# jlvdb/yet_another_wizz

Measured on AMD Instinct MI355X. Metric: candidate pairs/s, higher is better.
Workload: dtype f64

## Files before the change

### yet_another_wizz_amd/csrc/yawhip.hip

```cpp

#include <hip/hip_runtime.h>

#include <algorithm>
#include <numeric>
#include <chrono>
#include <climits>
#include <cmath>
#include <cstdio>
#include <cstdlib>
#include <cstring>
#include <memory>
#include <new>
#include <string>
#include <type_traits>
#include <utility>
#include <functional>
#include <vector>

#include "yawhip_internal.h"

using namespace yawhip_detail;

namespace {
constexpr int WG = 256;
constexpr int STAGE = 256;
constexpr int MSTAGE = 64;
constexpr int MAX_EDGES = 512;
constexpr int BAND_MIN_STREAM_RUN = 64;
constexpr int64_t SYNC_GRID_MIN_ITEMS = 400000;
constexpr int MAX_STRIP_REACH = 12;
constexpr int COUNT_FLUSH_MASK = (1 << 13) - 1;
constexpr int MERGED_FLUSH_MASK = (1 << 16) - 1;
constexpr double PAD_COORD = 4.0;

struct alignas(16) Obj {
    double x, y, z, w;
};

struct alignas(16) ObjF {
    float x, y, z, pad;
};

constexpr double FILTER_GUARD = 8.0 * 5.9604644775390625e-8;

inline double sep_angle(double rwin) { return 2.0 * std::asin(std::min(1.0, 0.5 * (rwin + 2e-9))); }

__device__ __forceinline__ double cap_lo64(double u, double c, double s) {
    const double ul = fmax(u - 1e-9, -1.0);
    return ul <= -c + 1e-12 ? -1.0 - 2e-9 : fma(ul, c, -sqrt(fmax(fma(-ul, ul, 1.0), 0.0)) * s) - 2e-9;
}
__device__ __forceinline__ double cap_hi64(double u, double c, double s) {
    const double uh = fmin(u + 1e-9, 1.0);
// ... 739 lines not shown
           (band_small_hist(weighted, nslots, hp) ? 0 : (size_t)nslots * hp * (weighted ? 8 : 4)) + 16;
}
typedef __attribute__((address_space(3))) unsigned char lds_byte;
__device__ __forceinline__ __attribute__((address_space(3))) void *lds_ptr(unsigned addr) { return (__attribute__((address_space(3))) void *)(size_t)addr; }
__device__ __forceinline__ double lds_f64(unsigned addr) { return *(const __attribute__((address_space(3))) double *)(size_t)addr; }
__device__ __forceinline__ int lds_i32(unsigned addr) { return *(const __attribute__((address_space(3))) int *)(size_t)addr; }

__device__ __forceinline__ int wave_max_nonneg(int v) {
    v = max(v, __builtin_amdgcn_update_dpp(0, v, 0x111, 0xf, 0xf, false));
    v = max(v, __builtin_amdgcn_update_dpp(0, v, 0x112, 0xf, 0xf, false));
    v = max(v, __builtin_amdgcn_update_dpp(0, v, 0x114, 0xf, 0xf, false));
    v = max(v, __builtin_amdgcn_update_dpp(0, v, 0x118, 0xf, 0xf, false));
    v = max(v, __builtin_amdgcn_update_dpp(0, v, 0x142, 0xa, 0xf, false));
    v = max(v, __builtin_amdgcn_update_dpp(0, v, 0x143, 0xc, 0xf, false));
    return __builtin_amdgcn_readlane(v, 63);
}

__device__ __forceinline__ unsigned int wave_sum_lane63(unsigned int v) {
    v += (unsigned int)__builtin_amdgcn_update_dpp(0, (int)v, 0x111, 0xf, 0xf, false);
    v += (unsigned int)__builtin_amdgcn_update_dpp(0, (int)v, 0x112, 0xf, 0xf, false);
    v += (unsigned int)__builtin_amdgcn_update_dpp(0, (int)v, 0x114, 0xf, 0xf, false);
    v += (unsigned int)__builtin_amdgcn_update_dpp(0, (int)v, 0x118, 0xf, 0xf, false);
    v += (unsigned int)__builtin_amdgcn_update_dpp(0, (int)v, 0x142, 0xa, 0xf, false);
    v += (unsigned int)__builtin_amdgcn_update_dpp(0, (int)v, 0x143, 0xc, 0xf, false);
    return v;
}

template <int R, int CAP, bool WEIGHTED, int NE, bool MERGED, bool UNI>
__global__ __launch_bounds__(64) void k_count_band(const DevTab *__restrict__ tabs, const Item *__restrict__ items, int n_bins,
                                                   int n_edges, const double *__restrict__ t,
                                                   const double *__restrict__ rwin_k, unsigned flush_mask, int hp_shift,
                                                   int batch_log2, unsigned long long *__restrict__ out_counts,
                                                   double *__restrict__ partials,
                                                   unsigned long long *__restrict__ counters) {
    using HistT = typename std::conditional<WEIGHTED, double, unsigned int>::type;
    constexpr bool NF1 = NE == 2;
    constexpr bool REG_EDGES = NE >= 2 && (!MERGED || UNI);
    constexpr bool NEED_THR = !REG_EDGES;
    constexpr int HB = WEIGHTED ? 3 : 2;
    using L = BandLds<CAP>;
    constexpr int LDS_X = L::X, LDS_K = L::K, LDS_Y = L::Y, LDS_H = L::H, LDS_Z = L::Z, LDS_H_BYTES = L::H_BYTES, BCOL = L::COL;
    __shared__ __attribute__((aligned(16))) unsigned char lds_fix[L::FIXED];
    extern __shared__ __attribute__((aligned(16))) unsigned char lds_dyn[];
    const int nkb = MERGED ? n_bins : 1;
    const int nf = NF1 ? 1 : n_edges - 1;
    const int nslots = nkb * nf;
    const int hp = 1 << hp_shift;
    double *sx = reinterpret_cast<double *>(lds_fix + LDS_X);
    double *sy = reinterpret_cast<double *>(lds_fix + LDS_Y);
    double *sz = reinterpret_cast<double *>(lds_fix + LDS_Z);
    int *sk = reinterpret_cast<int *>(lds_fix + LDS_K);
    unsigned char *p = lds_dyn;
    double *sw = reinterpret_cast<double *>(p); if (WEIGHTED) p += BCOL;
    constexpr bool ROW1 = !(MERGED && !UNI);
    const int thr_rows = ROW1 ? 1 : nkb;
    double *thr = reinterpret_cast<double *>(p); if (NEED_THR) p += (size_t)thr_rows * n_edges * sizeof(double);
    const bool small_hist = band_small_hist(WEIGHTED, nslots, hp);
    HistT *hist = reinterpret_cast<HistT *>(small_hist ? lds_fix + LDS_H : p);
    unsigned int *dummy = reinterpret_cast<unsigned int *>(lds_fix + LDS_H + LDS_H_BYTES);
    const int lane = threadIdx.x;
    const unsigned a_sx = (unsigned)(size_t)(lds_byte *)(lds_fix + LDS_X);
    const unsigned a_sw = (unsigned)(size_t)(lds_byte *)reinterpret_cast<unsigned char *>(sw);
    const unsigned a_cell = (unsigned)(size_t)(lds_byte *)reinterpret_cast<unsigned char *>(hist) + ((lane & (hp - 1)) << HB);
    const unsigned a_dummy = (unsigned)(size_t)(lds_byte *)reinterpret_cast<unsigned char *>(dummy + lane);
    const int ksh = hp_shift + HB;

    const unsigned long long n_kept = counters[0];
    const unsigned long long chunk = (n_kept + 7) >> 3;
    const unsigned long long n_batches = (chunk + (1ull << batch_log2) - 1) >> batch_log2;
    for (int e = lane; e < nslots * hp; e += 64) hist[e] = HistT(0);
    unsigned int cnt1 = 0;
    unsigned stage_no = 0;
    int pend_slot = -1;
    int thr_k = -1;
    auto flush_counts = [&](int slot_out) {
        if (NF1 && !MERGED) {
            if (lane == 0 && cnt1) atomicAdd(&out_counts[(int64_t)slot_out * nslots], (unsigned long long)cnt1);
            cnt1 = 0;
            return;
        }
        __syncthreads();
        for (int idx = lane; idx < nslots; idx += 64) {
            unsigned int c = 0;
            for (int h = 0; h < hp; ++h) {
                c += (unsigned int)hist[idx * hp + h];
                hist[idx * hp + h] = HistT(0);
            }
            if (c) atomicAdd(&out_counts[(int64_t)slot_out * nslots + idx], (unsigned long long)c);
        }
    };
    for (unsigned long long v = blockIdx.x;; v += gridDim.x) {
        if ((v >> 3) >= n_batches) break;
      for (unsigned long long j = (v >> 3) << batch_log2; j < (((v >> 3) + 1) << batch_log2) && j < chunk; ++j) {
        const unsigned long long ticket = (v & 7) * chunk + j;
        if (ticket >= n_kept) break;
        const Item it = items[ticket];
        const int o = item_orient(it), islot = item_slot(it);
        if (!WEIGHTED) {
            if (pend_slot >= 0 && pend_slot != islot) flush_counts(pend_slot);
            pend_slot = islot;
        }
        const DevTab c1 = tabs[o], c2 = tabs[3 + o];
        const int kfix = MERGED ? 0 : islot % n_bins;
        const double rwin = rwin_k[kfix];
        int64_t b0 = it.b0[0], nb_total = it.nb[0];

        __syncthreads();
        auto stage_in = [&](int64_t first, int n) {
            const gf64p gx = c1.x + b0 + first, gy = c1.y + b0 + first, gz = c1.z + b0 + first;
#pragma unroll
            for (int c = 0; c < (CAP + 127) / 128; ++c) {
                const unsigned e = (unsigned)(c * 128 + 2 * lane);
                if (e < (unsigned)n) {
                    __builtin_amdgcn_global_load_lds(gx + e, lds_ptr(a_sx + c * 1024), 16, 0, 0);
                    __builtin_amdgcn_global_load_lds(gy + e, lds_ptr(a_sx + (LDS_Y - LDS_X) + c * 1024), 16, 0, 0);
                    __builtin_amdgcn_global_load_lds(gz + e, lds_ptr(a_sx + (LDS_Z - LDS_X) + c * 1024), 16, 0, 0);
                    if (WEIGHTED && c1.w) __builtin_amdgcn_global_load_lds(c1.w + b0 + first + e, lds_ptr(a_sw + c * 1024), 16, 0, 0);
                }
            }
            if (MERGED) {
#pragma unroll
                for (int c = 0; c < (CAP + 255) / 256; ++c) {
                    const unsigned e = (unsigned)(c * 256 + 4 * lane);
                    if (e < (unsigned)n)
                        __builtin_amdgcn_global_load_lds(c1.k + b0 + first + e, lds_ptr(a_sx + (LDS_K - LDS_X) + c * 1024), 16, 0, 0);
                }
            }
// ... 179 lines not shown
                        if constexpr (!REG_EDGES) {
                            int c = 0;
                            for (int step = edge_top; step > 0; step >>= 1) {
                                const int probe = c + step;
                                c = sd > tk[probe < n_edges - 1 ? probe : n_edges - 1] ? probe : c;
                            }
                            slot += c;
                        }
                        const unsigned cell = ((unsigned)slot << ksh) + a_cell;
                        if constexpr (WEIGHTED)
                            (void)__hip_atomic_fetch_add((__attribute__((address_space(3))) double *)(size_t)cell, aw[r] * bw[r],
                                                         __ATOMIC_RELAXED, __HIP_MEMORY_SCOPE_WORKGROUP);
                        else
                            (void)__hip_atomic_fetch_add((__attribute__((address_space(3))) unsigned int *)(size_t)cell, 1u,
                                                         __ATOMIC_RELAXED, __HIP_MEMORY_SCOPE_WORKGROUP);
                    }
                }
                }
            }
            if (!WEIGHTED && (stage_no & flush_mask) == flush_mask) flush_counts(islot);
        }
        }
        if (WEIGHTED) flush_slab();
        for (int off = 32; off > 0; off >>= 1) nev += __shfl_down(nev, off, 64);
        if (lane == 0 && nev) atomicAdd(&counters[8 + 8 * (ticket & (EVAL_SLOTS - 1))], (unsigned long long)nev);
      }
        if (!WEIGHTED && pend_slot >= 0) {
            flush_counts(pend_slot);
            pend_slot = -1;
        }
    }
}

struct TicketMap {
    unsigned long long per_xcd;
    unsigned long long n_kept;
    unsigned long long seg_base;
    unsigned bs;
    bool segmented;
    __device__ __forceinline__ unsigned long long ticket(unsigned long long v) const {
        const unsigned long long j = v >> 3;
        if (segmented) return seg_base + j;
        return ((((j >> bs) << 3) + (v & 7)) << bs) + (j & ((1ull << bs) - 1ull));
    }
};
__device__ __forceinline__ TicketMap ticket_map(const unsigned long long *__restrict__ counters, unsigned long long seg_cap) {
    TicketMap m;
    m.segmented = seg_cap != 0;
    if (m.segmented) {
        const int seg = (int)(blockIdx.x % ITEM_SEGS);
        const unsigned long long n_seg = counters[ITEM_SEG_CTR(seg)];
        m.seg_base = (unsigned long long)seg * seg_cap;
        m.per_xcd = n_seg;
        m.n_kept = m.seg_base + n_seg;
        m.bs = 0;
        return m;
    }
    const unsigned long long n_kept = counters[0];
    m.n_kept = n_kept;
    m.seg_base = 0;
    const unsigned long long want = n_kept >> 7;
    int bs = want > 1 ? 63 - __builtin_clzll(want) : 0;
    bs = bs < 6 ? 6 : (bs > 12 ? 12 : bs);
    m.bs = (unsigned)bs;
    const unsigned long long nblocks = (n_kept + (1ull << bs) - 1ull) >> bs;
    m.per_xcd = ((nblocks + 7ull) >> 3) << bs;
    return m;
}

constexpr float PAD_COORD32 = 4.0f;
constexpr double BAND32_GUARD_SQRT = 2.1e-7;
__host__ __device__ constexpr int thr32_width(int ne) { return ne == 2 ? 4 : 2 * ne; }
__host__ __device__ inline size_t band32_lds(bool weighted, int cap, int nslots, int thr_rows, int ne) {
    return (size_t)3 * (cap + 4) * 4 + (weighted ? (size_t)(cap + 4) * 8 : 0) + (size_t)nslots * (weighted ? 8 : 4) +
           (size_t)thr_rows * thr32_width(ne) * 4 + 32;
}

template <int NT>
struct ExactEval {
    double s;
    double th[NT];
};
template <int NT>
__device__ __attribute__((noinline)) ExactEval<NT> band32_exact(gf64p lx, gf64p ly, gf64p lz, int64_t li, gf64p sx, gf64p sy, gf64p sz,
                                                               int64_t gi, const double *__restrict__ tk,
                                                               unsigned long long *__restrict__ counters) {
    atomicAdd(counters, 1ull);
    ExactEval<NT> r;
    const double ax = lx[li], ay = ly[li], az = lz[li], bx = sx[gi], by = sy[gi], bz = sz[gi];
#pragma unroll
    for (int e = 0; e < NT; ++e) r.th[e] = tk[e];
    const double dx = ax - bx, dy = ay - by, dz = az - bz;
    const double xx = dx * dx, yy = dy * dy, zz = dz * dz;
    const double sxy = xx + yy;
    r.s = sxy + zz;
    return r;
}

constexpr int B32_CAP = 320;
constexpr int B32_CAP_BIG = 512;
// ... 4 lines not shown
constexpr int B32_WAVES_LT = 1;
constexpr int band32_min_waves(int R, int CAP, bool WEIGHTED, int NE, bool UNI) {
    if (NE == 2 && UNI) {
        if (WEIGHTED) return R == 1 ? B32_WAVES_W1 : B32_WAVES_W;
        return CAP >= B32_CAP_BIG ? B32_WAVES_BIG : B32_WAVES_PLAIN;
    }
    return NE == 2 && !WEIGHTED ? B32_WAVES_LT : 1;
}

#define YAW_B32_NAME k_count_band32
#define YAW_B32_CH 3
#include "yawhip_band32.inc"
#undef YAW_B32_NAME
#undef YAW_B32_CH
#define YAW_B32_NAME k_count_band32_one
#define YAW_B32_CH 1
#include "yawhip_band32.inc"
#undef YAW_B32_NAME
#undef YAW_B32_CH

__host__ __device__ constexpr int fine32_width(int n_edges) { return 4 + 2 * n_edges; }
__host__ __device__ inline size_t band32_fine_lds(bool weighted, int cap, int nslots, int rows, int n_edges) {
    return (size_t)3 * (cap + 4) * 4 + (weighted ? (size_t)(cap + 2) * 8 : 0) + (size_t)nslots * (weighted ? 8 : 4) + 64 * 8 +
           (size_t)rows * fine32_width(n_edges) * 4 + 48;
}

template <int R, int CAP, bool WEIGHTED, bool MERGED, bool UNI>
__global__ __launch_bounds__(64) void k_count_band32_fine(const DevTab *__restrict__ tabs, const Item *__restrict__ items, int n_bins,
                                                          int n_edges, const double *__restrict__ t, const float *__restrict__ fine32,
                                                          const double *__restrict__ rwin_k, const float *__restrict__ ucap,
                                                          unsigned flush_mask, int swap,
                                                          unsigned long long *__restrict__ out_counts,
                                                          double *__restrict__ partials,
                                                          unsigned long long *__restrict__ counters, unsigned long long seg_cap) {
    using HistT = typename std::conditional<WEIGHTED, double, unsigned int>::type;
    constexpr int HB = WEIGHTED ? 3 : 2;
    extern __shared__ __attribute__((aligned(16))) unsigned char lds_dyn[];
    const int nkb = MERGED ? n_bins : 1;
    const int nf = n_edges - 1;
    const int nslots = nkb * nf;
    const int tw = fine32_width(n_edges);
    const int rows = UNI ? 1 : n_bins;
    unsigned char *p = lds_dyn;
    constexpr unsigned COLB = (CAP + 4) * 4;
    float *stage = reinterpret_cast<float *>(p); p += (size_t)3 * COLB;
    double *sw = reinterpret_cast<double *>(p); if (WEIGHTED) p += (size_t)(CAP + 2) * 8;
    HistT *hist = reinterpret_cast<HistT *>(p); p += (size_t)nslots * sizeof(HistT);
    p = reinterpret_cast<unsigned char *>(((size_t)p + 15) & ~(size_t)15);
    double *dummy = reinterpret_cast<double *>(p); p += 64 * 8;
    float *stab = reinterpret_cast<float *>(p);
    const int lane = threadIdx.x;
    const unsigned a_stage = (unsigned)(size_t)(lds_byte *)reinterpret_cast<unsigned char *>(stage);
    const unsigned a_sw = (unsigned)(size_t)(lds_byte *)reinterpret_cast<unsigned char *>(sw);
    const unsigned a_hist = (unsigned)(size_t)(lds_byte *)reinterpret_cast<unsigned char *>(hist);
    const unsigned a_dummy = (unsigned)(size_t)(lds_byte *)reinterpret_cast<unsigned char *>(dummy + lane);

    const TicketMap tmap = ticket_map(counters, seg_cap);
    const unsigned long long n_kept = tmap.n_kept;
    for (int e = lane; e < nslots; e += 64) hist[e] = HistT(0);
    for (int e = lane; e < rows * tw; e += 64) stab[e] = fine32[e];
    unsigned stage_no = 0;
    for (unsigned long long v = blockIdx.x;; v += gridDim.x) {
        if ((v >> 3) >= tmap.per_xcd) break;
        const unsigned long long ticket = tmap.ticket(v);
        if (ticket >= n_kept) continue;
        const Item it = items[ticket];
        const int o = item_orient(it), islot = item_slot(it);
        const DevTab cl = tabs[swap ? o : 3 + o], cs = tabs[swap ? 3 + o : o];
        const int kfix = MERGED ? 0 : islot % n_bins;
        const float rwin = (float)(rwin_k[kfix] * 1.000001 + 4e-7);
        int64_t b0 = it.b0[0], nb_total = it.nb[0];

        __syncthreads();
        auto stage_in = [&](int64_t first, int n) {
            const gf32p gx = cs.qx + b0 + first, gy = cs.qy + b0 + first, gz = cs.qz + b0 + first;
#pragma unroll
            for (int c = 0; c < (CAP + 255) / 256; ++c) {
                const unsigned e = (unsigned)(c * 256 + 4 * lane);
                if (e < (unsigned)n) {
                    __builtin_amdgcn_global_load_lds(gx + e, lds_ptr(a_stage + c * 1024), 16, 0, 0);
                    __builtin_amdgcn_global_load_lds(gy + e, lds_ptr(a_stage + COLB + c * 1024), 16, 0, 0);
                    __builtin_amdgcn_global_load_lds(gz + e, lds_ptr(a_stage + 2 * COLB + c * 1024), 16, 0, 0);
                }
            }
            if (WEIGHTED && cs.w) {
#pragma unroll
                for (int c = 0; c < (CAP + 127) / 128; ++c) {
                    const unsigned e = (unsigned)(c * 128 + 2 * lane);
                    if (e < (unsigned)n) __builtin_amdgcn_global_load_lds(cs.w + b0 + first + e, lds_ptr(a_sw + c * 1024), 16, 0, 0);
                }
            }
        };
        stage_in(0, (int)(nb_total < CAP ? nb_total : CAP));
        float ax[R], ay[R], az[R];
        double aw[R];
        int kb[R];
        int n_own = (int)it.na - lane * R;
// ... 394 lines not shown

}

namespace yawhip_detail {

CallKey::CallKey(const yawhip_ctx *ctx, const yawhip_catalog *c1, const yawhip_catalog *c2, int32_t n_jobs_, const int32_t *jobs_,
                 int32_t n_bins_, int32_t n_edges_, const double *t_, int32_t kernel_, bool want_counts_, bool want_sums_,
                 bool for_work_, int32_t n_dev_)
    : c1_uid(c1->uid), c2_uid(c2->uid), opt_gen(ctx->opt_gen), n_jobs(n_jobs_), n_bins(n_bins_), n_edges(n_edges_),
      kernel(kernel_), n_dev(n_dev_), want_counts(want_counts_), want_sums(want_sums_), for_work(for_work_), jobs(jobs_), t(t_) {
    auto mix = [this](uint64_t w) { hash = (hash ^ w) * 0x100000001b3ull; hash ^= hash >> 29; };
    for (uint64_t w : {c1_uid, c2_uid, opt_gen, (uint64_t)(uint32_t)n_jobs << 32 | (uint32_t)n_bins,
                       (uint64_t)(uint32_t)n_edges << 32 | (uint32_t)kernel,
                       (uint64_t)(uint32_t)n_dev << 32 | (uint64_t)(want_counts | want_sums << 1 | for_work << 2)})
        mix(w);
    for (size_t j = 0; j < (size_t)n_jobs; ++j) {
        uint64_t w;
        memcpy(&w, jobs + 2 * j, sizeof w);
        mix(w);
    }
    for (size_t i = 0; i < (size_t)n_bins * n_edges; ++i) {
        uint64_t w;
        memcpy(&w, t + i, sizeof w);
        mix(w);
    }
}

struct HostPlan {
    CallKey key;
    uint64_t stamp = 0;
    bool empty = false;
    bool split = false;
    int grid_div = 8;
    int R = 0, band_ne = 0, cap = 0, hp_shift = 0, lean_bins = 0, mode = 0, reach = 0, kernel = 0, nf = 0, n_orient = 0;
    bool band = false, band32 = false, band_fine = false, filter = false, lean = false, merged = false, run_unweighted = false,
         run_weighted = false, strip_items = false, swap = false, sweep = false, triple = false, uni = false, uniform_t = false,
         weighted = false;
    int64_t abytes = 0, cand = 0, n_items = 0, n_out = 0, n_pslots = 0, n_sjobs = 0, n_slots = 0, slab = 0, tile = 0;
    double rwin_max = 0.0;
    double cap_c = 1.0, cap_s = 0.0;
    size_t lds_band = 0, lds_merged = 0;
    unsigned char *d_in = nullptr;
    int32_t *d_jobs = nullptr;
    int64_t *d_prefix = nullptr, *d_cprefix = nullptr;
    double *d_t = nullptr, *d_rwin = nullptr;
    float *d_dthr = nullptr, *d_ucap = nullptr, *d_thr32 = nullptr;
    DevTab *d_tabs = nullptr;
    int64_t n_chunks = 0;
    ~HostPlan() { if (d_in) (void)hipFree(d_in); }
};

void drop_plans(yawhip_ctx *ctx, const yawhip_catalog *c) {
    for (size_t i = 0; i < ctx->plans.size();) {
        if (!c || ctx->plans[i]->key.c1_uid == c->uid || ctx->plans[i]->key.c2_uid == c->uid) {
            delete ctx->plans[i];
            ctx->plans[i] = ctx->plans.back();
            ctx->plans.pop_back();
        } else ++i;
    }
}

int check_call(const yawhip_ctx *ctx, const yawhip_catalog *c1, const yawhip_catalog *c2, int32_t n_jobs, const int32_t *jobs,
               int32_t n_bins, int32_t n_edges, const double *t) {
    if (!ctx || !c1 || !c2) return fail(YAWHIP_ERR_INVALID, "yawhip_count_pairs: NULL handle");
    if (n_jobs < 0 || n_bins <= 0 || n_edges < 2 || n_edges > MAX_EDGES || !t || (n_jobs > 0 && !jobs))
        return fail(YAWHIP_ERR_INVALID, "yawhip_count_pairs: bad sizes (n_jobs=%d n_bins=%d n_edges=%d, max edges %d)",
// ... 419 lines not shown
    }
    P.n_chunks = cprefix.empty() ? 0 : cprefix.back();
    const void *src[9] = {P.strip_items ? (const void *)job_recs.data() : (const void *)jobs, prefix.data(), t, dthr.data(),
                          rwin.data(), ucap.data(), thr32.data(), h_tabs, cprefix.data()};
    const size_t bytes[9] = {P.strip_items ? sizeof(JobRec) * (size_t)P.n_sjobs : sizeof(int32_t) * 2 * (size_t)n_jobs,
                             sizeof(int64_t) * ((size_t)P.n_pslots + 1), sizeof(double) * n_bins * n_edges, sizeof(float) * 3 * n_bins,
                             sizeof(double) * n_bins, sizeof(float) * 2 * n_bins, sizeof(float) * thr32.size(), sizeof h_tabs,
                             sizeof(int64_t) * cprefix.size()};
    size_t off[9], off_in = 0;
    for (int i = 0; i < 9; ++i) { off[i] = off_in; off_in = align16(off_in + bytes[i]); }
    std::vector<unsigned char> image(off_in, 0);
    for (int i = 0; i < 9; ++i)
        if (bytes[i]) memcpy(image.data() + off[i], src[i], bytes[i]);
    HIP_TRY(hipMalloc(reinterpret_cast<void **>(&P.d_in), std::max<size_t>(off_in, 16)));
    HIP_TRY(hipMemcpy(P.d_in, image.data(), off_in, hipMemcpyHostToDevice));
    P.d_jobs = reinterpret_cast<int32_t *>(P.d_in + off[0]);
    P.d_prefix = reinterpret_cast<int64_t *>(P.d_in + off[1]);
    P.d_t = reinterpret_cast<double *>(P.d_in + off[2]);
    P.d_dthr = reinterpret_cast<float *>(P.d_in + off[3]);
    P.d_rwin = reinterpret_cast<double *>(P.d_in + off[4]);
    P.d_ucap = reinterpret_cast<float *>(P.d_in + off[5]);
    P.d_thr32 = reinterpret_cast<float *>(P.d_in + off[6]);
    P.d_tabs = reinterpret_cast<DevTab *>(P.d_in + off[7]);
    P.d_cprefix = reinterpret_cast<int64_t *>(P.d_in + off[8]);
    P.n_orient = (L1[0] ? 1 : 0) + (L1[1] ? 1 : 0) + (L1[2] ? 1 : 0);
    double skew = 1.0;
    for (const StripLayout *const *LX : {L1, L2})
        for (int o = 0; o < 3; ++o)
            if (LX[o] && LX[o]->built) {
                const yawhip_catalog *cx = LX == L1 ? c1 : c2;
                const double runs = (double)std::max<int64_t>(LX[o]->h_vbase[(size_t)LX[o]->n_groups], 1);
                skew = std::max(skew, LX[o]->obj_run / std::max((double)cx->n / runs, 1.0));
            }
    P.grid_div = ctx->band_grid_div > 0 ? ctx->band_grid_div : (skew > 2.0 ? 4 : (P.mode == 3 ? 16 : 8));
    if (g_trace.on) fprintf(stderr, "[yawhip trace] run skew %.2f -> grid / %d\n", skew, P.grid_div);
    return YAWHIP_OK;
}

int make_plan(yawhip_ctx *ctx, const yawhip_catalog *c1, const yawhip_catalog *c2, int32_t n_jobs, const int32_t *jobs,
              int32_t n_bins, int32_t n_edges, const double *t, int32_t kernel, bool want_counts, bool want_sums, bool for_work,
              HostPlan &P) {
    Planner pl{ctx, c1, c2, n_jobs, jobs, n_bins, n_edges, t, for_work, P};
    int rc = pl.kernel_and_sizes(kernel, want_counts, want_sums);
    if (rc == YAWHIP_OK && !P.empty) rc = pl.layouts();
    if (rc == YAWHIP_OK && !P.empty) rc = pl.tile_and_stage();
    if (rc == YAWHIP_OK && !P.empty) rc = pl.histogram();
    if (rc == YAWHIP_OK && !P.empty) rc = pl.items();
    if (rc == YAWHIP_OK && !P.empty && !P.split) rc = pl.tables();
    if (rc == YAWHIP_OK) g_trace.mark("planned");
    return rc;
}

}

namespace yawhip_detail {

int count_enqueue(yawhip_ctx *ctx, const yawhip_catalog *c1, const yawhip_catalog *c2, int32_t n_jobs,
                  const int32_t *jobs, int32_t n_bins, int32_t n_edges, const double *t, int32_t kernel,
                  bool want_counts, bool want_sums, int64_t *job_work, CallState &cs, bool fetch_results) {
    cs = CallState{};
    cs.wall0 = std::chrono::steady_clock::now();
    g_trace.mark("enqueue");
    cs.want_counts = want_counts;
    cs.want_sums = want_sums;
    HIP_TRY(hipSetDevice(ctx->device));
    CallKey key(ctx, c1, c2, n_jobs, jobs, n_bins, n_edges, t, kernel, want_counts, want_sums, job_work != nullptr);
    HostPlan *plan = nullptr;
    for (HostPlan *cand_plan : ctx->plans)
// ... 91 lines not shown
            HIP_TRY(hipStreamSynchronize(ctx->stream));
            n_items = (int64_t)reinterpret_cast<unsigned long long *>(ctx->out.h)[0];
        }
    }
    if (job_work) {
        HIP_TRY(ctx->d_jobwork.reserve((size_t)n_jobs));
        HIP_TRY(hipMemsetAsync(ctx->d_jobwork.ptr, 0, sizeof(unsigned long long) * (size_t)n_jobs, ctx->stream));
        if (n_pot > 0) {
            hipLaunchKernelGGL(k_item_work, dim3((unsigned)((n_pot + 255) / 256)), dim3(256), 0, ctx->stream, ctx->d_items.ptr,
                               ctx->d_ctr, P.merged ? 1 : n_bins, ctx->d_jobwork.ptr);
            HIP_TRY(hipGetLastError());
        }
        HIP_TRY(hipMemcpyAsync(job_work, ctx->d_jobwork.ptr, sizeof(int64_t) * (size_t)n_jobs, hipMemcpyDeviceToHost,
                               ctx->stream));
        HIP_TRY(hipStreamSynchronize(ctx->stream));
        return YAWHIP_OK;
    }
    auto reduce_partials = [&]() -> hipError_t {
        const int64_t n_oslots = P.n_pslots, values = P.slab, n_chunks = P.n_chunks;
        hipError_t er = ctx->d_chunk_sums.reserve((size_t)std::max<int64_t>(n_chunks, 1) * values);
        if (er != hipSuccess) return er;
        const int thr = 256;
        const bool all_kept = !(P.run_weighted && P.sweep);
        if (n_chunks > 0)
            hipLaunchKernelGGL(k_reduce_chunks, dim3((unsigned)((n_chunks * values + thr - 1) / thr)), dim3(thr), 0, ctx->stream,
                               ctx->d_partials.ptr, all_kept ? nullptr : ctx->d_kept.ptr, P.d_prefix, P.d_cprefix,
                               (int)n_oslots, (int)values, ctx->d_chunk_sums.ptr, ctx->d_ctr);
        hipLaunchKernelGGL(k_reduce_slots, dim3((unsigned)((n_oslots * values + thr - 1) / thr)), dim3(thr), 0, ctx->stream,
                           ctx->d_chunk_sums.ptr, P.d_cprefix, (int)n_oslots, (int)values, ctx->d_sums,
                           n_chunks > 0 ? nullptr : ctx->d_ctr);
        return hipGetLastError();
    };
    if (!cs.stamps) HIP_TRY(hipEventRecord(ctx->evc0, ctx->stream));
    int64_t grid = P.strip_items && n_pot > 65536 ? n_pot / P.grid_div : n_pot;
    const int batch_log2 = ctx->band_batch_log2 >= 0 ? ctx->band_batch_log2 : 0;
    if (!P.run_weighted) grid = std::max<int64_t>(grid >> batch_log2, 8);
    grid = std::min<int64_t>((grid + 7) & ~7ll, 1ll << 22);
    const dim3 band_grid((unsigned)grid), wave(64);
    int flush_log2 = ctx->flush_log2;
    while (flush_log2 > 0 && ((uint64_t)64 * P.R * 2 * P.cap << flush_log2) >= (1ull << 32)) --flush_log2;
    const unsigned flush_mask = (1u << flush_log2) - 1u;
    const std::pair<int, int> stage{P.R, P.cap};
    const std::pair<bool, bool> rows{P.merged, P.uni};
    auto launch_band32 = [&](bool wgt) -> hipError_t {
        const size_t lds = band32_lds(P.weighted, P.cap, P.lean_bins * P.nf, P.merged && !P.uniform_t ? n_bins : 0, n_edges);
        const bool one_chunk = P.triple || !P.strip_items;
        return pick<Bool<false>, Bool<true>>(wgt, [&](auto w) {
            return pick<Int<4>, Int<3>, Int<2>>(n_edges, [&](auto ne) {
                return pick<Rows<true, false>, Rows<true, true>, Rows<false, true>>(rows, [&](auto r) {
                    return pick<Stage<4, B32_CAP_BIG>, Stage<2, B32_CAP_BIG>, Stage<2, B32_CAP>, Stage<1, B32_CAP>>(stage, [&](auto s) {
                        using S = decltype(s);
                        using M = decltype(r);
                        auto kern = one_chunk ? k_count_band32_one<S::R, S::CAP, w, ne, M::MERGED, M::UNI>
                                              : k_count_band32<S::R, S::CAP, w, ne, M::MERGED, M::UNI>;
                        cs.variant[w] = variant_code(one_chunk ? VF_BAND32_ONE : VF_BAND32, S::R, S::CAP, w, ne, M::MERGED, M::UNI);
                        return launch(kern, band_grid, wave, lds, ctx->stream, P.d_tabs, ctx->d_items.ptr, n_bins, P.d_t,
                                      P.d_thr32, P.d_rwin, P.d_ucap, flush_mask, P.swap ? 1 : 0, ctx->d_counts,
                                      ctx->d_partials.ptr, ctx->d_ctr, seg_cap);
                    });
                });
            });
        });
    };
    auto launch_band64 = [&](bool wgt) -> hipError_t {
        return pick<Bool<false>, Bool<true>>(wgt, [&](auto w) {
            return pick<Int<0>, Int<4>, Int<3>, Int<2>>(P.band_ne, [&](auto ne) {
                return pick<Rows<true, false>, Rows<true, true>, Rows<false, true>>(rows, [&](auto r) {
                    return pick<Stage<4, BCAP_MID>, Stage<2, BCAP_MID>, Stage<2, BCAP>, Stage<1, BCAP>>(stage, [&](auto s) {
                        using S = decltype(s);
                        using M = decltype(r);
                        cs.variant[w] = variant_code(VF_BAND, S::R, S::CAP, w, ne, M::MERGED, M::UNI);
                        return launch(k_count_band<S::R, S::CAP, w, ne, M::MERGED, M::UNI>, band_grid, wave, P.lds_band, ctx->stream,
                                      P.d_tabs, ctx->d_items.ptr, n_bins, n_edges, P.d_t, P.d_rwin, flush_mask,
                                      P.hp_shift, w ? 0 : batch_log2, ctx->d_counts, ctx->d_partials.ptr, ctx->d_ctr);
                    });
                });
            });
        });
    };
    auto launch_fine = [&](bool wgt) -> hipError_t {
        const size_t lds = band32_fine_lds(P.weighted, P.cap, P.lean_bins * P.nf, P.uniform_t ? 1 : n_bins, n_edges);
        return pick<Bool<false>, Bool<true>>(wgt, [&](auto w) {
            return pick<Rows<true, false>, Rows<true, true>, Rows<false, false>, Rows<false, true>>(rows, [&](auto r) {
                return pick<Stage<4, BCAP_MID>, Stage<2, BCAP_MID>, Stage<2, BCAP>, Stage<1, BCAP>>(stage, [&](auto s) {
                    using S = decltype(s);
                    using M = decltype(r);
                    cs.variant[w] = variant_code(VF_BAND32_FINE, S::R, S::CAP, w, 0, M::MERGED, M::UNI);
                    return launch(k_count_band32_fine<S::R, S::CAP, w, M::MERGED, M::UNI>, band_grid, wave, lds, ctx->stream,
                                  P.d_tabs, ctx->d_items.ptr, n_bins, n_edges, P.d_t, P.d_thr32, P.d_rwin,
                                  P.d_ucap, flush_mask, P.swap ? 1 : 0, ctx->d_counts, ctx->d_partials.ptr, ctx->d_ctr, seg_cap);
                });
            });
        });
    };
    auto in_pieces = [&](int wg, auto &&launch_at) -> hipError_t {
        const int64_t max_grid = (1ll << 31) / wg;
        for (int64_t base = 0; base < n_items; base += max_grid) {
            const hipError_t e = launch_at(dim3((unsigned)std::min(max_grid, n_items - base)), base);
            if (e != hipSuccess) return e;
        }
        return hipSuccess;
    };
    auto launch_lean = [&](bool wgt) -> hipError_t {
        return pick<Bool<false>, Bool<true>>(wgt, [&](auto w) {
            return pick<Bool<false>, Bool<true>>(P.nf == 1, [&](auto nf1) {
                return pick<Bool<false>, Bool<true>>(P.merged, [&](auto m) {
                    return pick<Int<4>, Int<2>, Int<1>>(P.R, [&](auto r) {
                        cs.variant[w] = variant_code(r <= 2 ? VF_MERGED_OCC8 : VF_MERGED,
                                                      r, 0, w, 0, m, false, false, false, nf1);
                        return in_pieces(MWG, [&](dim3 g, int64_t base) {
                            return launch(pick_count_merged<r, w, nf1, m>(), g, dim3(MWG), P.lds_merged, ctx->stream, P.d_tabs,
                                          ctx->d_items.ptr, n_bins, n_edges, P.d_t, P.d_dthr, P.d_rwin, base,
                                          ctx->d_counts, ctx->d_partials.ptr, ctx->d_ctr);
                        });
                    });
                });
            });
        });
    };
    const size_t lds_fixed = 2 * STAGE * (sizeof(Obj) + sizeof(ObjF)) + (size_t)((n_edges + 1) & ~1) * sizeof(double);
    auto lds_for = [&](bool w, bool priv) { return lds_fixed + (size_t)P.nf * (priv ? WG : 1) * (w ? 8 : 4); };
    auto launch_plain = [&](bool wgt) -> hipError_t {
        const bool priv = lds_for(wgt, true) <= (size_t)ctx->lds_limit;
// ... 296 lines not shown
```

### yet_another_wizz_amd/csrc/yawhip_api.hip

```cpp

#include <hip/hip_runtime.h>

#include <algorithm>
#include <atomic>
#include <climits>
#include <cstdarg>
#include <cstdint>
#include <cstdio>
#include <cstring>
#include <functional>
#include <new>
#include <string>
#include <system_error>
#include <thread>
#include <utility>
#include <vector>

#include "yawhip_internal.h"
#include "yawhip_hist.h"
#include "yawhip_random.h"

namespace yawhip_detail {

thread_local Trace g_trace;
// ... 160 lines not shown
        number(&yawhip_ctx::triple_runs);
    } else if (!strcmp(key, "item_segments")) {
        flag(&yawhip_ctx::item_segments);
    } else if (!strcmp(key, "spin_wait")) {
        flag(&yawhip_ctx::spin_wait);
    } else if (!strcmp(key, "band_cap")) {
        if (const int rc = check_band_cap(value)) return rc;
        number(&yawhip_ctx::band_cap);
    } else if (!strcmp(key, "strip_grid")) {
        if (value != 0 && value != 1) return fail(YAWHIP_ERR_INVALID, "strip_grid must be 0 (linear in v) or 1 (latitude)");
        number(&yawhip_ctx::strip_grid);
    } else if (!strcmp(key, "band_trim")) {
        if (value != 0 && value != 1) return fail(YAWHIP_ERR_INVALID, "band_trim must be 0 or 1");
        number(&yawhip_ctx::band_trim);
    } else if (!strcmp(key, "strip_width_micro")) {
        if (value != 0 && (value < 1000 || value > 2000000))
            return fail(YAWHIP_ERR_INVALID, "strip_width_micro must be 0 (off) or in [1e3, 2e6]");
        set = [=](yawhip_ctx &c) { c.strip_width = (double)value * 1e-6; };
    } else if (!strcmp(key, "seg_strips_min_run")) {
        if (value < 1) return fail(YAWHIP_ERR_INVALID, "seg_strips_min_run must be >= 1");
        set = [=](yawhip_ctx &c) { c.seg_min_run = (int)std::min<int64_t>(value, INT32_MAX); };
    } else if (!strcmp(key, "seg_strips")) {
        flag(&yawhip_ctx::seg_strips);
    } else if (!strcmp(key, "debug_no_hits")) {
        flag(&yawhip_ctx::debug_no_hits);
    } else if (!strcmp(key, "auto_orient")) {
        flag(&yawhip_ctx::auto_orient);
    } else if (!strcmp(key, "slab_budget_bytes")) {
        if (value < 4096) return fail(YAWHIP_ERR_INVALID, "slab_budget_bytes must be >= 4096");
        set = [=](yawhip_ctx &c) { c.slab_budget = value; };
    } else if (!strcmp(key, "band_grid_div")) {
        if (value < 0 || value > 64) return fail(YAWHIP_ERR_INVALID, "band_grid_div must be 0 (auto) or in [1, 64]");
        number(&yawhip_ctx::band_grid_div);
    } else if (!strcmp(key, "flush_stages_log2")) {
        if (value < 0 || value > 17) return fail(YAWHIP_ERR_INVALID, "flush_stages_log2 must be in [0, 17]");
        number(&yawhip_ctx::flush_log2);
    } else if (!strcmp(key, "band_fp32")) {
        flag(&yawhip_ctx::band_fp32);
    } else if (!strcmp(key, "hist_chunk_log2")) {
        if (value < 8 || value > 30) return fail(YAWHIP_ERR_INVALID, "hist_chunk_log2 must be in [8, 30]");
        number(&yawhip_ctx::hist_chunk_log2);
    } else if (!strcmp(key, "kernel")) {
        if (value < YAWHIP_KERNEL_AUTO || value > YAWHIP_KERNEL_BAND)
            return fail(YAWHIP_ERR_INVALID, "unknown kernel id %lld", (long long)value);
        number(&yawhip_ctx::default_kernel);
    } else {
        return fail(YAWHIP_ERR_INVALID, "unknown option '%s'", key);
    }
    std::vector<yawhip_ctx *> devices(ctx->peers);
    devices.push_back(ctx);
    for (yawhip_ctx *c : devices) {
        ++c->opt_gen;
        drop_plans(c, nullptr);
        set(*c);
    }
    return YAWHIP_OK;
}

int yawhip_ctx_create_multi(const int *device_ids, int n_devices, yawhip_ctx **out) {
    if (!out) return fail(YAWHIP_ERR_INVALID, "yawhip_ctx_create_multi: out is NULL");
    *out = nullptr;
    if (!device_ids || n_devices < 1 || n_devices > 64) return fail(YAWHIP_ERR_INVALID, "yawhip_ctx_create_multi: 1 to 64 device ids");
    yawhip_ctx *ctx = nullptr;
    int rc = yawhip_ctx_create(device_ids[0], &ctx);
    if (rc != YAWHIP_OK) return rc;
    for (int i = 1; i < n_devices; ++i) {
// ... 223 lines not shown
```

### yet_another_wizz_amd/csrc/yawhip_band32.inc

```
template <int R, int CAP, bool WEIGHTED, int NE, bool MERGED, bool UNI>
__global__ __launch_bounds__(64, band32_min_waves(R, CAP, WEIGHTED, NE, UNI))
void YAW_B32_NAME(const DevTab *__restrict__ tabs, const Item *__restrict__ items, int n_bins,
                  const double *__restrict__ t, const float *__restrict__ thr32,
                  const double *__restrict__ rwin_k, const float *__restrict__ ucap,
                  unsigned flush_mask, int swap,
                  unsigned long long *__restrict__ out_counts,
                  double *__restrict__ partials,
                  unsigned long long *__restrict__ counters, unsigned long long seg_cap) {
    static_assert(NE >= 2 && NE <= 4, "edges per bin");
    constexpr int CH = YAW_B32_CH;
    constexpr bool PAIRS = R == 1 && CH == 1;
    constexpr int NS = PAIRS ? 2 : R;
    static_assert(CH == 1 || CH == 3, "chunks per round");
    static_assert(CAP % 4 == 0, "stage capacity");
    using HistT = typename std::conditional<WEIGHTED, double, unsigned int>::type;
    constexpr int NC = NE == 2 ? 1 : NE;
    constexpr int NF = NE - 1;
    constexpr int TW = thr32_width(NE);
    constexpr bool LANE_THR = MERGED && !UNI;
    extern __shared__ __attribute__((aligned(16))) unsigned char lds_dyn[];
    const int nkb = MERGED ? n_bins : 1;
    const int nslots = nkb * NF;
    unsigned char *p = lds_dyn;
    constexpr unsigned COLB = (CAP + 4) * 4;
    float *stage = reinterpret_cast<float *>(p); p += (size_t)3 * COLB;
    double *sw = reinterpret_cast<double *>(p); if (WEIGHTED) p += (size_t)(CAP + 4) * 8;
    HistT *hist = reinterpret_cast<HistT *>(p); p += (size_t)nslots * sizeof(HistT);
    p = reinterpret_cast<unsigned char *>(((size_t)p + 15) & ~(size_t)15);
    float *sthr = reinterpret_cast<float *>(p);
    const int lane = threadIdx.x;
    const unsigned a_stage = (unsigned)(size_t)(lds_byte *)reinterpret_cast<unsigned char *>(stage);
    const unsigned a_sw = (unsigned)(size_t)(lds_byte *)reinterpret_cast<unsigned char *>(sw);
    const unsigned a_hist = (unsigned)(size_t)(lds_byte *)reinterpret_cast<unsigned char *>(hist);

    const TicketMap tmap = ticket_map(counters, seg_cap);
    const unsigned long long n_kept = tmap.n_kept;
    for (int e = lane; e < nslots; e += 64) hist[e] = HistT(0);
    if (LANE_THR)
        for (int e = lane; e < n_bins * TW; e += 64) sthr[e] = thr32[e];
    unsigned round_no = 0;
    for (unsigned long long v = blockIdx.x;; v += gridDim.x) {
        if ((v >> 3) >= tmap.per_xcd) break;
        const unsigned long long ticket = tmap.ticket(v);
        if (ticket >= n_kept) continue;
        const Item it = items[ticket];
        const int o = item_orient(it), islot = item_slot(it);
        const DevTab cl = tabs[swap ? o : 3 + o], cs = tabs[swap ? 3 + o : o];
        const int kfix = MERGED ? 0 : islot % n_bins;
        const float rwin = (float)(rwin_k[kfix] * 1.000001 + 4e-7);

        int win = 0;
        int64_t win_off = 0;
        int64_t cb[CH];
        int cn[CH], co[CH];
        int nch = 0;
        auto next_round = [&]() {
            nch = 0;
            int used = 0;
#pragma unroll
            for (int c = 0; c < CH; ++c) {
                cb[c] = 0; cn[c] = 0; co[c] = 0;
                if (win < it.nwin && nch == c) {
                    const int64_t wb = win == 0 ? it.b0[0] : (win == 1 ? it.b0[1] : it.b0[2]);
                    const int64_t rem = (int64_t)(win == 0 ? it.nb[0] : (win == 1 ? it.nb[1] : it.nb[2])) - win_off;
                    if (rem + 1 <= (int64_t)(CAP - used)) {
                        cb[c] = wb + win_off; cn[c] = (int)rem; co[c] = used;
                        used += ((int)rem + 1 + 3) & ~3;
                        ++win; win_off = 0; ++nch;
                    } else if (c == 0) {
                        cb[c] = wb + win_off; cn[c] = CAP - 4; co[c] = 0;
                        used = CAP;
                        win_off += CAP - 4; ++nch;
                    }
                }
            }
        };
// ... 356 lines not shown
```

### yet_another_wizz_amd/csrc/yawhip_internal.h

```cpp
#ifndef YAWHIP_INTERNAL_H
#define YAWHIP_INTERNAL_H
#include <hip/hip_runtime.h>

#include <chrono>
#include <cstdint>
#include <cstdio>
#include <cstdlib>
#include <cstring>
#include <functional>
#include <string>
#include <utility>
#include <vector>

#include "yawhip.h"
#include "yawhip_healpix.h"
#include "yawhip_sort.h"

#pragma GCC visibility push(hidden)

namespace yawhip_detail {
struct Trace {
    bool on = getenv("YAWHIP_TRACE") != nullptr;
    int n = 0;
    const char *name[32];
// ... 229 lines not shown
    int64_t n_groups = 0;
    int64_t device_bytes = 0;
    double obj_run = 0.0;
    double same_bin = 0.0;
    void release() {
        for (void *ptr : {(void *)x, (void *)y, (void *)z, (void *)w, (void *)k, (void *)q, (void *)off, (void *)d_vbase, (void *)d_slo,
                          (void *)d_tiles[0], (void *)d_tiles[1], (void *)d_tiles[2], (void *)d_tile_rec[0], (void *)d_tile_rec[1],
                          (void *)d_tile_rec[2], (void *)d_grid, (void *)q3, (void *)w3, (void *)idx3, (void *)pos3, (void *)off3, (void *)d_grid3})
            if (ptr) (void)hipFree(ptr);
        q3 = nullptr; w3 = nullptr; idx3 = nullptr; pos3 = nullptr; off3 = nullptr; d_grid3 = nullptr; triples = false;
        x = y = z = w = nullptr; k = nullptr; q = nullptr; off = d_vbase = d_slo = nullptr;
        d_tiles[0] = d_tiles[1] = d_tiles[2] = nullptr;
        d_tile_rec[0] = d_tile_rec[1] = d_tile_rec[2] = nullptr;
        d_grid = nullptr;
        built = false;
    }
};

}

struct yawhip_ctx : yawhip_detail::CallBufs {
    int device = 0;
    hipStream_t stream = nullptr;
    int tile_r = 0;
    int hist_copies_log2 = -1;
    int band_batch_log2 = -1;
    int band_cap = 0;
    int seg_strips = 1;
    int seg_min_run = yawhip_detail::SEG_STRIPS_MIN_RUN;
    int debug_no_hits = 0;
    int auto_orient = 1;
    int64_t slab_budget = 1ll << 30;
    int band_grid_div = 0;
    int flush_log2 = 17;
    int spin_wait = 1;
    int item_segments = 1;
    int half_bands = 1;
    int triple_runs = 1;
    int band_fp32 = 1;
    double strip_width = 0.005;
    int strip_grid = 1;
    int band_trim = 1;
    int default_kernel = YAWHIP_KERNEL_AUTO;
    int hist_chunk_log2 = 23;
    int lds_limit = 160 * 1024;
    int n_cu = 256;
    yawhip_detail::DevBuf<unsigned long long> d_jobwork;
    yawhip_detail::DevBuf<double> d_full;
    yawhip_detail::DevBuf<int32_t> d_rowidx;
    std::vector<yawhip_ctx *> peers;
    struct Plan {
        yawhip_detail::CallKey key;
        std::vector<std::vector<int32_t>> parts;
    } plan;
    yawsort::Workspace sort_ws;
    yawpix::Workspace pix_ws;
    yawhip_detail::CallBufs parked[yawhip_detail::MAX_BATCH];
    int slot = 0;
    uint64_t opt_gen = 1;
    uint64_t plan_clock = 0;
    std::vector<yawhip_detail::HostPlan *> plans;
};

struct yawhip_catalog {
    yawhip_ctx *ctx = nullptr;
    uint64_t uid = 0;
// ... 84 lines not shown
```

Baseline: 32510000 billion.

## Taper band-kernel work rounds so tail rounds shrink across fewer workgroups

Replaces the plain grid-stride ticket loop in the band kernels with a tapered schedule. After full-width rounds, successive rounds use progressively fewer workgroups, so the final partial round is spread more evenly and tail imbalance shrinks. For non-clustered inputs the grid divisor also rises from 8 to 12 when tapering is on, launching fewer but longer-lived workgroups. The ticket mapping moves to a shared header and the schedule values are made wave-uniform with readfirstlane. The cost is extra index arithmetic and a schedule that could mis-cover or unbalance tickets if the round math is off.

```diff
diff --git a/yet_another_wizz_amd/csrc/yawhip.hip b/yet_another_wizz_amd/csrc/yawhip.hip
--- a/yet_another_wizz_amd/csrc/yawhip.hip
+++ b/yet_another_wizz_amd/csrc/yawhip.hip
@@ -18,6 +18,7 @@
 #include <vector>
 
 #include "yawhip_internal.h"
+#include "yawhip_tickets.h"
 
 using namespace yawhip_detail;
 
@@ -823,7 +824,7 @@
                                                    const double *__restrict__ rwin_k, unsigned flush_mask, int hp_shift,
                                                    int batch_log2, unsigned long long *__restrict__ out_counts,
                                                    double *__restrict__ partials,
-                                                   unsigned long long *__restrict__ counters) {
+                                                   unsigned long long *__restrict__ counters, int taper) {
     using HistT = typename std::conditional<WEIGHTED, double, unsigned int>::type;
     constexpr bool NF1 = NE == 2;
     constexpr bool REG_EDGES = NE >= 2 && (!MERGED || UNI);
@@ -880,10 +881,11 @@
             if (c) atomicAdd(&out_counts[(int64_t)slot_out * nslots + idx], (unsigned long long)c);
         }
     };
-    for (unsigned long long v = blockIdx.x;; v += gridDim.x) {
-        if ((v >> 3) >= n_batches) break;
-      for (unsigned long long j = (v >> 3) << batch_log2; j < (((v >> 3) + 1) << batch_log2) && j < chunk; ++j) {
-        const unsigned long long ticket = (v & 7) * chunk + j;
+    const TaperMap rounds = taper_map(gridDim.x >> 3, n_batches, taper != 0);
+    const unsigned wg = blockIdx.x >> 3, xcd = blockIdx.x & 7u;
+    for (TaperWalk tw = taper_begin(rounds, wg); taper_more(tw); taper_next(rounds, tw)) {
+      for (unsigned long long j = tw.index << batch_log2; j < ((tw.index + 1) << batch_log2) && j < chunk; ++j) {
+        const unsigned long long ticket = (unsigned long long)xcd * chunk + j;
         if (ticket >= n_kept) break;
         const Item it = items[ticket];
         const int o = item_orient(it), islot = item_slot(it);
@@ -1129,40 +1131,32 @@
     }
 }
 
-struct TicketMap {
-    unsigned long long per_xcd;
-    unsigned long long n_kept;
-    unsigned long long seg_base;
-    unsigned bs;
-    bool segmented;
-    __device__ __forceinline__ unsigned long long ticket(unsigned long long v) const {
-        const unsigned long long j = v >> 3;
-        if (segmented) return seg_base + j;
-        return ((((j >> bs) << 3) + (v & 7)) << bs) + (j & ((1ull << bs) - 1ull));
-    }
+constexpr int BAND_TAPER_AUTO = 1;
+constexpr int BAND_DIV_TAPER = 12;
+struct BandSchedule {
+    TicketMap tmap;
+    TaperMap rounds;
+    TaperWalk begin;
 };
-__device__ __forceinline__ TicketMap ticket_map(const unsigned long long *__restrict__ counters, unsigned long long seg_cap) {
-    TicketMap m;
-    m.segmented = seg_cap != 0;
-    if (m.segmented) {
-        const int seg = (int)(blockIdx.x % ITEM_SEGS);
-        const unsigned long long n_seg = counters[ITEM_SEG_CTR(seg)];
-        m.seg_base = (unsigned long long)seg * seg_cap;
-        m.per_xcd = n_seg;
-        m.n_kept = m.seg_base + n_seg;
-        m.bs = 0;
-        return m;
-    }
-    const unsigned long long n_kept = counters[0];
-    m.n_kept = n_kept;
-    m.seg_base = 0;
-    const unsigned long long want = n_kept >> 7;
-    int bs = want > 1 ? 63 - __builtin_clzll(want) : 0;
-    bs = bs < 6 ? 6 : (bs > 12 ? 12 : bs);
-    m.bs = (unsigned)bs;
-    const unsigned long long nblocks = (n_kept + (1ull << bs) - 1ull) >> bs;
-    m.per_xcd = ((nblocks + 7ull) >> 3) << bs;
-    return m;
+__device__ __forceinline__ BandSchedule band_schedule(const unsigned long long *__restrict__ counters, unsigned long long seg_cap,
+                                                      int taper) {
+    BandSchedule s;
+    if (seg_cap != 0) {
+        const unsigned seg = blockIdx.x % ITEM_SEGS;
+        s.tmap = ticket_map_segment(seg, counters[ITEM_SEG_CTR((int)seg)], seg_cap);
+    } else {
+        s.tmap = ticket_map_dealt(blockIdx.x & 7u, counters[0]);
+    }
+    s.rounds = taper_map(gridDim.x >> 3, s.tmap.per_xcd, taper != 0);
+    s.begin = taper_begin(s.rounds, blockIdx.x >> 3);
+    s.begin.index += s.tmap.first;
+    auto uni = [](unsigned v) { return (unsigned)__builtin_amdgcn_readfirstlane((int)v); };
+    s.rounds.D = uni(s.rounds.D);
+    s.begin.width = uni(s.begin.width);
+    s.begin.k = (int)uni((unsigned)s.begin.k);
+    s.begin.end = (int)uni((unsigned)s.begin.end);
+    s.begin.index = ((unsigned long long)uni((unsigned)(s.begin.index >> 32)) << 32) | uni((unsigned)s.begin.index);
+    return s;
 }
 
 constexpr float PAD_COORD32 = 4.0f;
@@ -1233,7 +1227,7 @@
                                                           unsigned flush_mask, int swap,
                                                           unsigned long long *__restrict__ out_counts,
                                                           double *__restrict__ partials,
-                                                          unsigned long long *__restrict__ counters, unsigned long long seg_cap) {
+                                                          unsigned long long *__restrict__ counters, unsigned long long seg_cap, int taper) {
     using HistT = typename std::conditional<WEIGHTED, double, unsigned int>::type;
     constexpr int HB = WEIGHTED ? 3 : 2;
     extern __shared__ __attribute__((aligned(16))) unsigned char lds_dyn[];
@@ -1256,14 +1250,13 @@
     const unsigned a_hist = (unsigned)(size_t)(lds_byte *)reinterpret_cast<unsigned char *>(hist);
     const unsigned a_dummy = (unsigned)(size_t)(lds_byte *)reinterpret_cast<unsigned char *>(dummy + lane);
 
-    const TicketMap tmap = ticket_map(counters, seg_cap);
-    const unsigned long long n_kept = tmap.n_kept;
+    const BandSchedule sched = band_schedule(counters, seg_cap, taper);
+    const unsigned long long n_kept = sched.tmap.n_kept;
     for (int e = lane; e < nslots; e += 64) hist[e] = HistT(0);
     for (int e = lane; e < rows * tw; e += 64) stab[e] = fine32[e];
     unsigned stage_no = 0;
-    for (unsigned long long v = blockIdx.x;; v += gridDim.x) {
-        if ((v >> 3) >= tmap.per_xcd) break;
-        const unsigned long long ticket = tmap.ticket(v);
+    for (TaperWalk tw_ = sched.begin; taper_more(tw_); taper_next(sched.rounds, tw_)) {
+        const unsigned long long ticket = sched.tmap.ticket(tw_.index);
         if (ticket >= n_kept) continue;
         const Item it = items[ticket];
         const int o = item_orient(it), islot = item_slot(it);
@@ -1724,6 +1717,7 @@
     bool empty = false;
     bool split = false;
     int grid_div = 8;
+    int taper = 0;
     int R = 0, band_ne = 0, cap = 0, hp_shift = 0, lean_bins = 0, mode = 0, reach = 0, kernel = 0, nf = 0, n_orient = 0;
     bool band = false, band32 = false, band_fine = false, filter = false, lean = false, merged = false, run_unweighted = false,
          run_weighted = false, strip_items = false, swap = false, sweep = false, triple = false, uni = false, uniform_t = false,
@@ -2209,8 +2203,12 @@
                 const double runs = (double)std::max<int64_t>(LX[o]->h_vbase[(size_t)LX[o]->n_groups], 1);
                 skew = std::max(skew, LX[o]->obj_run / std::max((double)cx->n / runs, 1.0));
             }
-    P.grid_div = ctx->band_grid_div > 0 ? ctx->band_grid_div : (skew > 2.0 ? 4 : (P.mode == 3 ? 16 : 8));
-    if (g_trace.on) fprintf(stderr, "[yawhip trace] run skew %.2f -> grid / %d\n", skew, P.grid_div);
+    const bool clustered = skew > 2.0;
+    P.taper = ctx->band_taper >= 0 ? ctx->band_taper : (clustered || P.mode == 3 ? 0 : BAND_TAPER_AUTO);
+    const int div_uniform = P.mode == 3 ? 16 : (P.taper ? BAND_DIV_TAPER : 8);
+    P.grid_div = ctx->band_grid_div > 0 ? ctx->band_grid_div : (clustered ? 4 : div_uniform);
+    if (g_trace.on)
+        fprintf(stderr, "[yawhip trace] run skew %.2f -> grid / %d, %s rounds\n", skew, P.grid_div, P.taper ? "tapered" : "plain");
     return YAWHIP_OK;
 }
 
@@ -2368,7 +2366,10 @@
         return hipGetLastError();
     };
     if (!cs.stamps) HIP_TRY(hipEventRecord(ctx->evc0, ctx->stream));
-    int64_t grid = P.strip_items && n_pot > 65536 ? n_pot / P.grid_div : n_pot;
+    int64_t grid = P.strip_items && n_pot > ctx->band_grid_floor ? std::max<int64_t>(n_pot / P.grid_div, 1) : n_pot;
+    const int taper = P.taper;
+    if (g_trace.on && P.band)
+        fprintf(stderr, "[yawhip trace] %lld potential items -> %lld band workgroups\n", (long long)n_pot, (long long)((grid + 7) & ~7ll));
     const int batch_log2 = ctx->band_batch_log2 >= 0 ? ctx->band_batch_log2 : 0;
     if (!P.run_weighted) grid = std::max<int64_t>(grid >> batch_log2, 8);
     grid = std::min<int64_t>((grid + 7) & ~7ll, 1ll << 22);
@@ -2392,7 +2393,7 @@
                         cs.variant[w] = variant_code(one_chunk ? VF_BAND32_ONE : VF_BAND32, S::R, S::CAP, w, ne, M::MERGED, M::UNI);
                         return launch(kern, band_grid, wave, lds, ctx->stream, P.d_tabs, ctx->d_items.ptr, n_bins, P.d_t,
                                       P.d_thr32, P.d_rwin, P.d_ucap, flush_mask, P.swap ? 1 : 0, ctx->d_counts,
-                                      ctx->d_partials.ptr, ctx->d_ctr, seg_cap);
+                                      ctx->d_partials.ptr, ctx->d_ctr, seg_cap, taper);
                     });
                 });
             });
@@ -2408,7 +2409,7 @@
                         cs.variant[w] = variant_code(VF_BAND, S::R, S::CAP, w, ne, M::MERGED, M::UNI);
                         return launch(k_count_band<S::R, S::CAP, w, ne, M::MERGED, M::UNI>, band_grid, wave, P.lds_band, ctx->stream,
                                       P.d_tabs, ctx->d_items.ptr, n_bins, n_edges, P.d_t, P.d_rwin, flush_mask,
-                                      P.hp_shift, w ? 0 : batch_log2, ctx->d_counts, ctx->d_partials.ptr, ctx->d_ctr);
+                                      P.hp_shift, w ? 0 : batch_log2, ctx->d_counts, ctx->d_partials.ptr, ctx->d_ctr, taper);
                     });
                 });
             });
@@ -2424,7 +2425,7 @@
                     cs.variant[w] = variant_code(VF_BAND32_FINE, S::R, S::CAP, w, 0, M::MERGED, M::UNI);
                     return launch(k_count_band32_fine<S::R, S::CAP, w, M::MERGED, M::UNI>, band_grid, wave, lds, ctx->stream,
                                   P.d_tabs, ctx->d_items.ptr, n_bins, n_edges, P.d_t, P.d_thr32, P.d_rwin,
-                                  P.d_ucap, flush_mask, P.swap ? 1 : 0, ctx->d_counts, ctx->d_partials.ptr, ctx->d_ctr, seg_cap);
+                                  P.d_ucap, flush_mask, P.swap ? 1 : 0, ctx->d_counts, ctx->d_partials.ptr, ctx->d_ctr, seg_cap, taper);
                 });
             });
         });
diff --git a/yet_another_wizz_amd/csrc/yawhip_api.hip b/yet_another_wizz_amd/csrc/yawhip_api.hip
--- a/yet_another_wizz_amd/csrc/yawhip_api.hip
+++ b/yet_another_wizz_amd/csrc/yawhip_api.hip
@@ -216,6 +216,12 @@
     } else if (!strcmp(key, "band_grid_div")) {
         if (value < 0 || value > 64) return fail(YAWHIP_ERR_INVALID, "band_grid_div must be 0 (auto) or in [1, 64]");
         number(&yawhip_ctx::band_grid_div);
+    } else if (!strcmp(key, "band_taper")) {
+        if (value < -1 || value > 1) return fail(YAWHIP_ERR_INVALID, "band_taper must be -1 (auto), 0 or 1");
+        number(&yawhip_ctx::band_taper);
+    } else if (!strcmp(key, "band_grid_floor")) {
+        if (value < 0) return fail(YAWHIP_ERR_INVALID, "band_grid_floor must be >= 0");
+        set = [=](yawhip_ctx &c) { c.band_grid_floor = value; };
     } else if (!strcmp(key, "flush_stages_log2")) {
         if (value < 0 || value > 17) return fail(YAWHIP_ERR_INVALID, "flush_stages_log2 must be in [0, 17]");
         number(&yawhip_ctx::flush_log2);
diff --git a/yet_another_wizz_amd/csrc/yawhip_band32.inc b/yet_another_wizz_amd/csrc/yawhip_band32.inc
--- a/yet_another_wizz_amd/csrc/yawhip_band32.inc
+++ b/yet_another_wizz_amd/csrc/yawhip_band32.inc
@@ -6,7 +6,7 @@
                   unsigned flush_mask, int swap,
                   unsigned long long *__restrict__ out_counts,
                   double *__restrict__ partials,
-                  unsigned long long *__restrict__ counters, unsigned long long seg_cap) {
+                  unsigned long long *__restrict__ counters, unsigned long long seg_cap, int taper) {
     static_assert(NE >= 2 && NE <= 4, "edges per bin");
     constexpr int CH = YAW_B32_CH;
     constexpr bool PAIRS = R == 1 && CH == 1;
@@ -33,15 +33,14 @@
     const unsigned a_sw = (unsigned)(size_t)(lds_byte *)reinterpret_cast<unsigned char *>(sw);
     const unsigned a_hist = (unsigned)(size_t)(lds_byte *)reinterpret_cast<unsigned char *>(hist);
 
-    const TicketMap tmap = ticket_map(counters, seg_cap);
-    const unsigned long long n_kept = tmap.n_kept;
+    const BandSchedule sched = band_schedule(counters, seg_cap, taper);
+    const unsigned long long n_kept = sched.tmap.n_kept;
     for (int e = lane; e < nslots; e += 64) hist[e] = HistT(0);
     if (LANE_THR)
         for (int e = lane; e < n_bins * TW; e += 64) sthr[e] = thr32[e];
     unsigned round_no = 0;
-    for (unsigned long long v = blockIdx.x;; v += gridDim.x) {
-        if ((v >> 3) >= tmap.per_xcd) break;
-        const unsigned long long ticket = tmap.ticket(v);
+    for (TaperWalk tw = sched.begin; taper_more(tw); taper_next(sched.rounds, tw)) {
+        const unsigned long long ticket = sched.tmap.ticket(tw.index);
         if (ticket >= n_kept) continue;
         const Item it = items[ticket];
         const int o = item_orient(it), islot = item_slot(it);
diff --git a/yet_another_wizz_amd/csrc/yawhip_internal.h b/yet_another_wizz_amd/csrc/yawhip_internal.h
--- a/yet_another_wizz_amd/csrc/yawhip_internal.h
+++ b/yet_another_wizz_amd/csrc/yawhip_internal.h
@@ -285,6 +285,8 @@
     int auto_orient = 1;
     int64_t slab_budget = 1ll << 30;
     int band_grid_div = 0;
+    int band_taper = -1;
+    int64_t band_grid_floor = 65536;
     int flush_log2 = 17;
     int spin_wait = 1;
     int item_segments = 1;
diff --git a/yet_another_wizz_amd/csrc/yawhip_tickets.h b/yet_another_wizz_amd/csrc/yawhip_tickets.h
--- /dev/null
+++ b/yet_another_wizz_amd/csrc/yawhip_tickets.h
@@ -0,0 +1,86 @@
+#pragma once
+
+#ifndef YAW_HD
+#if defined(__HIPCC__) || defined(__CUDACC__)
+#define YAW_HD __host__ __device__ inline
+#else
+#define YAW_HD inline
+#endif
+#endif
+
+struct TicketMap {
+    unsigned long long per_xcd;
+    unsigned long long n_kept;
+    unsigned long long first;
+    unsigned bs;
+    unsigned xcd;
+    YAW_HD unsigned long long ticket(unsigned long long b) const { return b + ((((b >> bs) * 7ull) + xcd) << bs); }
+};
+YAW_HD TicketMap ticket_map_segment(unsigned seg, unsigned long long n_seg, unsigned long long seg_cap) {
+    TicketMap m;
+    m.first = (unsigned long long)seg * seg_cap;
+    m.per_xcd = n_seg;
+    m.n_kept = m.first + n_seg;
+    m.bs = 63;
+    m.xcd = 0;
+    return m;
+}
+YAW_HD TicketMap ticket_map_dealt(unsigned xcd, unsigned long long n_kept) {
+    TicketMap m;
+    m.n_kept = n_kept;
+    m.first = 0;
+    m.xcd = xcd;
+    const unsigned long long want = n_kept >> 7;
+    int bs = want > 1 ? 63 - __builtin_clzll(want) : 0;
+    bs = bs < 6 ? 6 : (bs > 12 ? 12 : bs);
+    m.bs = (unsigned)bs;
+    const unsigned long long nblocks = (n_kept + (1ull << bs) - 1ull) >> bs;
+    m.per_xcd = ((nblocks + 7ull) >> 3) << bs;
+    return m;
+}
+
+#ifndef YAW_TAPER_R_MAX
+#define YAW_TAPER_R_MAX 16
+#endif
+struct TaperMap {
+    unsigned G;
+    unsigned D;
+    unsigned F, Rt;
+};
+YAW_HD TaperMap taper_map(unsigned G, unsigned long long n, bool tapered) {
+    TaperMap m;
+    m.G = G; m.D = 0; m.Rt = 0;
+    unsigned long long covered = 0;
+    if (tapered) {
+        const unsigned long long q = (n + G - 1) / G;
+        unsigned long long rt = q >= 2 ? 2 * q - 2 : 0;
+        const unsigned long long cap = G - 1 < (unsigned)YAW_TAPER_R_MAX ? G - 1 : (unsigned)YAW_TAPER_R_MAX;
+        rt = rt > cap ? cap : rt;
+        m.Rt = (unsigned)rt;
+        m.D = G / (unsigned)(rt + 1);
+        covered = rt * G - (unsigned long long)m.D * (rt * (rt + 1) / 2);
+    }
+    m.F = n > covered ? (unsigned)((n - covered + G - 1) / G) : 0u;
+    return m;
+}
+struct TaperWalk {
+    unsigned long long index;
+    unsigned width;
+    int k;
+    int end;
+};
+YAW_HD TaperWalk taper_begin(const TaperMap &m, unsigned j) {
+    TaperWalk w;
+    w.k = -(int)m.F;
+    w.width = m.F ? m.G : m.G - m.D;
+    w.index = j;
+    const unsigned reach = m.Rt ? (m.G - 1 - j) / m.D : 0u;
+    w.end = (int)(reach < m.Rt ? reach : m.Rt);
+    return w;
+}
+YAW_HD bool taper_more(const TaperWalk &w) { return w.k < w.end; }
+YAW_HD void taper_next(const TaperMap &m, TaperWalk &w) {
+    w.index += w.width;
+    ++w.k;
+    if (w.k >= 0) w.width -= m.D;
+}
```

After: 33270000 billion (median of 2 runs). No clear change (+2.3%).
